# cisco-system-traffic-generator/trex-emu

Measured on AMD Instinct MI355X. Metric: Mpkt/s device-resident rx parse+classify, 1M×64B batch, 1/2/4/8 MI355X, higher is better.
Workload: dtype u8; 1 GPU; B: 1M x 64B untagged IPv4/UDP, 1 ns / 1 client; frames_per_gpu=1048576, frame_bytes_per_gpu=67108864, parallelism=frame shards x1, replicated tables, no collective, tables=replicated, descriptors=keyed (EMURX_DESC_KEYED owner keys, as the device framing walk writes them), table_bytes_per_gpu=109664256, streams=2, batches=8, input_bytes_per_batch=79691840, input_reuse_distance_bytes=637534720

## Files before the change

### include/emu_rx.h

```cpp
#ifndef EMU_RX_H
#define EMU_RX_H

#include <stddef.h>
#include <stdint.h>

#ifdef __cplusplus
extern "C" {
#endif

#define EMURX_ABI_VERSION 6

#define EMURX_OK 0
#define EMURX_EINVAL (-22)
#define EMURX_ENOMEM (-12)
#define EMURX_EEXIST (-17)
#define EMURX_ENOENT (-2)
#define EMURX_EDEVICE (-5)
#define EMURX_ENOSPC (-28)

#define EMURX_ID_NONE 0xFFFFFFFFu

#define EMURX_MAX_FRAME 9216u
#define EMURX_ZMQ_MAGIC 0xBEEFu

// ... 325 lines not shown
    EMURX_LRN_NONE = 0,
    EMURX_LRN_ARP_REQ = 1, EMURX_LRN_ARP_REPLY = 2, EMURX_LRN_ND_NS = 3, EMURX_LRN_ND_NA = 4,
    EMURX_LRN_HOST = 5
};
#define EMURX_LRNK_ARP 1u
#define EMURX_LRNK_ND  2u
#define EMURX_LRNK_ALL 3u
#define EMURX_LRN_INFO_WORDS 8
uint32_t emurx_learn_max_events(const emurx_t* h);
int emurx_learn_dev(emurx_t* h, const uint8_t* d_frames, const emurx_desc* d_desc,
                    const emurx_rec* d_rec, uint32_t n, uint32_t kinds,
                    emurx_learn_ev* d_ev, uint32_t ev_cap,
                    uint8_t* d_outcome, uint64_t* d_info, void* stream);

void emurx_hist_to_counters(const uint64_t hist[2 * EMURX_HIST_BINS], emurx_counters* out);
void emurx_hist_fold(const uint64_t* shards, uint64_t out[2 * EMURX_HIST_BINS]);

int emurx_set_timing(emurx_t* h, uint32_t slots, uint32_t stride);
int emurx_kernel_times(emurx_t* h, float* batch_ms, uint32_t cap, uint32_t* n_out);

const char* emurx_build_id(void);

uint32_t emurx_last_stage(const emurx_t* h);
int32_t emurx_last_txz(const emurx_t* h);

int emurx_copy_ceiling_dev(void* d_dst, const void* d_src, size_t bytes, void* stream);

#define EMURX_MAX_PARTS 8
typedef struct emurx_route_rec {
    emurx_rec rec;
    uint32_t src_index;
    uint32_t src_rank;
} emurx_route_rec;

uint32_t emurx_ns_owner(const uint8_t key[12], uint32_t n_parts);
uint8_t emurx_owner_key(const uint8_t key[12]);
int emurx_desc_keys_dev(emurx_t* h, const uint8_t* d_frames, emurx_desc* d_desc, uint32_t n, void* stream);
int emurx_route_dev(emurx_t* h, const emurx_rec* d_rec, uint32_t n, uint32_t n_parts, uint32_t my_rank,
                    uint32_t cap, emurx_route_rec* d_send, uint32_t* d_send_count, void* stream);
int emurx_classify_route_dev(emurx_t* h, const uint8_t* d_frames, const emurx_desc* d_desc, uint32_t n,
                             const emurx_dev_out* out, uint32_t n_parts, uint32_t my_rank, uint32_t cap,
                             emurx_route_rec* d_send, uint32_t* d_send_count, void* stream);

#define EMURX_TAIL_SHARDS 64u
#define EMURX_TAIL_CURSOR_STRIDE 64u
#define EMURX_LOOKUP_REGION_BYTES(cap, tail_cap) \
// ... 36 lines not shown
```

### trex-emu_amd/csrc/emurx_api.cpp

```cpp
#include <hip/hip_runtime.h>

#include <algorithm>
#include <atomic>
#include <chrono>
#include <array>
#include <cstdio>
#include <cstdlib>
#include <cstring>
#include <new>
#include <string>
#include <vector>

#include "../../include/emu_rx.h"
#include "emurx_kernels.h"
#include "emurx_mirror.h"
#include "emurx_tables.h"

using emurx_host::Blocks;
using emurx_host::Hash;
using emurx_host::Mirror;

namespace {

uint16_t be16(const uint8_t* p) { return (uint16_t)((p[0] << 8) | p[1]); }
// ... 133 lines not shown
    uint32_t txz_calls = 0, txz_last_copy = 0, txz_every = 8, txz_same = 0;
    int last_txz = -1;
    DevBuf<uint8_t> d_rsp;
    DevBuf<uint8_t> d_lrn;
    bool lrn_dirty = false;

    struct RouteScratch {
        hipStream_t st = nullptr;
        bool used = false;
        hipEvent_t done = nullptr;
        DevBuf<uint32_t> cnt, grp, goff;
        DevBuf<uint32_t> tcur;
        void release() {
            cnt.release(); grp.release(); goff.release(); tcur.release();
            if (done) (void)hipEventDestroy(done);
            done = nullptr;
        }
    };
    static constexpr size_t kRouteSets = 4;
    RouteScratch route[kRouteSets];
    uint32_t route_next = 0;

    DevBuf<uint32_t> d_stage_fb;
    PinBuf<uint32_t> stage_fb;
    uint32_t stage_gen = 0, stage_mode = 0;
    bool stage_copy = false, stage_pending = false;
    uint32_t stage_copy_gen = 0;
    uint32_t stage_every = 8, stage_same = 0;
    hipEvent_t stage_ev = nullptr;
    uint32_t stage_bytes = emurx::kStageWide;
    bool stage_tight_ok = false;
    uint32_t last_stage = 0;

    emurx_comm_state* comm = nullptr;

    std::vector<hipEvent_t> ev;
    uint32_t slots = 0, ev_head = 0, ev_count = 0, stride = 1, batch_seq = 0;

    emurx_dev_tables tables() const {
        using namespace emurx_host;
        emurx_dev_tables T{};
        T.ns_tab = d_tab[kTabNs].p;
        T.ns_info = d_nsinfo.p;
        T.mac_tab = d_tab[kTabMac].p;
        T.ip4_tab = d_tab[kTabIp4].p;
        T.ip6_tab = d_tab[kTabIp6].p;
// ... 207 lines not shown
    return EMURX_HIP_OK(hipEventRecord(r->done, st)) ? EMURX_OK : EMURX_EDEVICE;
}

int not_capturing(hipStream_t st) {
    hipStreamCaptureStatus cs = hipStreamCaptureStatusNone;
    if (!EMURX_HIP_OK(hipStreamIsCapturing(st, &cs))) return EMURX_EDEVICE;
    return cs == hipStreamCaptureStatusNone ? EMURX_OK : EMURX_EINVAL;
}

int run_dev(emurx_t* h, const uint8_t* frames, const emurx_desc* desc, uint32_t n, const emurx_dev_out* out,
            hipStream_t st, int kind, const emurx_route_args* rt) {
    int rc;
    if ((rc = not_capturing(st))) return rc;
    if (kind == 1 && (rc = prepare_read(h, st))) return rc;
    emurx_dev_tables T = h->tables();
    const hipEvent_t* ev = nullptr;
    if (h->slots && (h->batch_seq++ % h->stride) == 0) {
        const uint32_t s = h->ev_head;
        ev = &h->ev[2 * s];
        h->ev_head = (s + 1) % h->slots;
        h->ev_count = std::min(h->ev_count + 1, h->slots);
    }
    const uint32_t stage = choose_stage(h);
    int r = emurx_launch_batch(frames, desc, n, T, kind, *out, st, ev, stage, h->d_stage_fb.p, h->stage_gen, rt);
    if (!r) r = stage_copy_back(h, st);
    return r ? EMURX_EDEVICE : EMURX_OK;
}

int check_batch_args(emurx_t* h, const uint8_t* frames, const emurx_desc* desc, uint32_t n,
                     const emurx_dev_out* out) {
    if (!h || !out || !out->hist || (n && (!frames || !desc))) return EMURX_EINVAL;
    if (((uintptr_t)frames & 15) || ((uintptr_t)desc & 7)) return EMURX_EINVAL;
    if (n > h->cfg.max_frames) return EMURX_ENOMEM;
    if (out->qlist && out->qcap < queue_cap(n)) return EMURX_EINVAL;
    return bind(h);
}

int ingest_buffer(emurx_t* h, uint32_t slot, size_t bytes, uint8_t** buf) {
    IngestSlot& s = h->ing[slot];
    if (s.pending || bytes > 0xFFFFFFFFull - 64) return EMURX_EINVAL;
    if (s.h_buf.alloc(bytes + 64) || s.d_buf.alloc(bytes + 64)) return EMURX_ENOMEM;
    *buf = s.h_buf.p;
    return EMURX_OK;
}

bool small_fits(const uint32_t* ctl, uint32_t nmsg, uint32_t n, uint32_t max_tiles, uint32_t trange[EMURX_SMALL_TILES]) {
    if (nmsg > EMURX_SMALL_MSGS || n > std::min<uint32_t>(max_tiles, EMURX_SMALL_TILES) * EMURX_QUEUE_TILE) return false;
// ... 102 lines not shown
        if (emurx_launch_ingest_small(s.h_buf.p, ctl, nmsg, n, h->tables(), s.h_rec.p, s.h_desc.p, s.h_qlist.p,
                                      s.h_stat.p, s.h_qoff.p, s.h_hist.p, s.d_qseg.p, s.d_tcnt.p, s.d_hsmall.p,
                                      s.d_ticket.p, s.h_done.p, (s.seq + 1) & 0x7fffffffu,
                                      h->spin_base_us > 0 ? (uint32_t)((h->spin_base_us + 1e-4 * (double)end) * h->wall_khz / 1000.0) : 0u,
                                      trange, st) ||
            !EMURX_HIP_OK(hipEventRecord(s.done, st)))
            return EMURX_EDEVICE;
        s.seq = (s.seq + 1) & 0x7fffffffu;
        s.small = true;
        s.pending = true;
        s.nmsg = nmsg;
        s.slots = n;
        return EMURX_OK;
    }
    const auto H2D = hipMemcpyHostToDevice, D2H = hipMemcpyDeviceToHost;
    bool ok = EMURX_HIP_OK(hipMemcpyAsync(s.d_ctl.p, ctl, ((size_t)3 * nmsg + 1) * 4, H2D, st));
    if (end) ok = ok && EMURX_HIP_OK(hipMemcpyAsync(s.d_buf.p, s.h_buf.p, end, H2D, st));
    if (!ok) return EMURX_EDEVICE;
    if (emurx_launch_zmq_walk(s.d_buf.p, s.d_ctl.p, nmsg, s.d_desc.p, s.d_stat.p, st)) return EMURX_EDEVICE;
    if (n) {
        const emurx_dev_out o{s.d_rec.p, s.d_qlist.p, (uint32_t)qcap, s.d_tile_cnt.p, s.d_hist.p};
        const uint32_t stage = choose_stage(h);
        if (emurx_launch_batch(s.d_buf.p, s.d_desc.p, n, h->tables(), true, o, st, nullptr, stage,
                               h->d_stage_fb.p, h->stage_gen) ||
            stage_copy_back(h, st))
            return EMURX_EDEVICE;
    }
    if (emurx_launch_queue_pack(s.d_qlist.p, (uint32_t)qcap, s.d_tile_cnt.p, n, s.d_seg_off.p, s.d_packed.p,
                                s.d_qoff.p, s.d_hist.p, s.d_hist_out.p, st))
        return EMURX_EDEVICE;
    ok = EMURX_HIP_OK(hipMemcpyAsync(s.h_res.p, s.d_res.p, s.res_bytes, D2H, st)) &&
         EMURX_HIP_OK(hipEventRecord(s.done, st));
    if (!ok) return EMURX_EDEVICE;
    s.small = false;
    s.pending = true;
    s.nmsg = nmsg;
    s.slots = n;
    return EMURX_OK;
}

bool spin_done(const uint32_t* word, uint32_t seq) {
    const volatile uint32_t* w = word;
    const auto t0 = std::chrono::steady_clock::now();
    for (uint32_t k = 1;; ++k) {
        if ((*w & 0x7fffffffu) == seq) {
            std::atomic_thread_fence(std::memory_order_acquire);
            return true;
// ... 88 lines not shown
}

int emurx_open(const emurx_cfg* cfg, emurx_t** out) {
    if (!cfg || !out || cfg->max_ns == 0 || cfg->max_clients == 0 || cfg->max_frames == 0) return EMURX_EINVAL;
    emurx_t* h = new (std::nothrow) emurx_ctx();
    if (!h) return EMURX_ENOMEM;
    h->cfg = *cfg;
    if (h->cfg.max_bytes == 0) h->cfg.max_bytes = 1u << 20;
    h->host_only = cfg->device < 0;
    try {
        h->m.open(cfg->max_ns, cfg->max_clients);
    } catch (...) {
        delete h;
        return EMURX_ENOMEM;
    }
    if (h->host_only) {
        *out = h;
        return EMURX_OK;
    }
    int rc = bind(h);
    if (rc) { delete h; return rc; }
    if (!EMURX_HIP_OK(hipStreamCreate(&h->stream))) { delete h; return EMURX_EDEVICE; }
    if (const char* e = getenv("EMURX_STAGE")) h->stage_mode = !strcmp(e, "wide") ? 1 : !strcmp(e, "narrow") ? 2 : !strcmp(e, "tight") ? 3 : 0;
    if (const char* e = getenv("EMURX_INGEST_SMALL")) h->ingest_small = strcmp(e, "0") != 0;
    if (const char* e = getenv("EMURX_TXZ"))
        h->txz_mode = !strcmp(e, "wide") ? EMURX_TXZ_WIDE : !strcmp(e, "narrow") ? EMURX_TXZ_NARROW
                    : !strcmp(e, "long") ? EMURX_TXZ_LONG : -1;
    if (const char* e = getenv("EMURX_INGEST_SPIN")) h->ingest_spin = strcmp(e, "0") != 0;
    {
        int khz = 100000;
        if (EMURX_HIP_OK(hipDeviceGetAttribute(&khz, hipDeviceAttributeWallClockRate, cfg->device)) && khz > 0)
            h->wall_khz = (uint32_t)khz;
        if (const char* e = getenv("EMURX_INGEST_SPIN_US")) h->spin_base_us = std::min(std::max(0.0, strtod(e, nullptr)), 1e6);
        const uint32_t cap = emurx_ingest_small_capacity(cfg->device);
        h->small_tiles = std::min<uint32_t>(EMURX_SMALL_TILES, cap);
    }
    if (h->stage_fb.alloc(256) || h->d_stage_fb.alloc(256) ||
        !EMURX_HIP_OK(hipEventCreateWithFlags(&h->stage_ev, hipEventDisableTiming)) ||
        !EMURX_HIP_OK(hipEventCreateWithFlags(&h->ship_ev, hipEventDisableTiming)) ||
        !EMURX_HIP_OK(hipMemset(h->d_stage_fb.p, 0, 256 * sizeof(uint32_t)))) {
        emurx_close(h);
        return EMURX_ENOMEM;
    }
    for (auto& s : h->ring)
        if (!EMURX_HIP_OK(hipEventCreateWithFlags(&s.ev, hipEventDisableTiming))) {
            emurx_close(h);
            return EMURX_EDEVICE;
        }
    memset(h->stage_fb.p, 0, 256 * sizeof(uint32_t));
    if (h->d_lrn.alloc(emurx_lrn_scratch_bytes(cfg->max_frames)) ||
        !EMURX_HIP_OK(hipMemset(h->d_lrn.p, 0, (size_t)emurx_lrn_slots(cfg->max_frames) * 16))) {
        emurx_close(h);
        return EMURX_ENOMEM;
    }
    emurx_t::RouteScratch* rs = nullptr;
    if ((rc = ship_tables(h, h->stream)) || (rc = route_scratch(h, cfg->max_frames, h->stream, &rs)) == EMURX_ENOMEM) {
        emurx_close(h);
        return rc ? rc : EMURX_ENOMEM;
    }
    *out = h;
    return EMURX_OK;
}

// ... 396 lines not shown
    for (int b = 0; b < 2 * EMURX_HIST_BINS; ++b) out[b] = 0;
    if (!shards) return;
    for (int s = 0; s < EMURX_HIST_SHARDS; ++s)
        for (int b = 0; b < 2 * EMURX_HIST_BINS; ++b) out[b] += shards[(size_t)s * 2 * EMURX_HIST_BINS + b];
}

int emurx_set_timing(emurx_t* h, uint32_t slots, uint32_t stride) {
    if (!h) return EMURX_EINVAL;
    int rc = bind(h);
    if (rc) return rc;
    (void)hipDeviceSynchronize();
    for (auto& e : h->ev)
        if (e) (void)hipEventDestroy(e);
    h->ev.assign((size_t)slots * 2, nullptr);
    for (auto& e : h->ev)
        if (!EMURX_HIP_OK(hipEventCreateWithFlags(&e, hipEventDisableSystemFence))) { h->slots = 0; return EMURX_EDEVICE; }
    h->slots = slots;
    h->stride = stride ? stride : 1;
    h->ev_head = h->ev_count = h->batch_seq = 0;
    return EMURX_OK;
}

uint32_t emurx_last_stage(const emurx_t* h) { return h ? h->last_stage : 0; }
int32_t emurx_last_txz(const emurx_t* h) {
    if (!h || h->last_txz < 0) return -1;
    return h->last_txz == EMURX_TXZ_NARROW ? 4608 : h->last_txz == EMURX_TXZ_LONG ? 0 : 6144;
}

int emurx_kernel_times(emurx_t* h, float* batch_ms, uint32_t cap, uint32_t* n_out) {
    if (!h || !n_out || (cap && !batch_ms)) return EMURX_EINVAL;
    *n_out = 0;
    if (!h->slots || !h->ev_count) return EMURX_OK;
    int rc = bind(h);
    if (rc) return rc;
    const uint32_t last = (h->ev_head + h->slots - 1) % h->slots;
    if (!EMURX_HIP_OK(hipEventSynchronize(h->ev[2 * last + 1]))) return EMURX_EDEVICE;
    const uint32_t n = std::min(h->ev_count, cap);
    const uint32_t first = (h->ev_head + h->slots - h->ev_count) % h->slots;
    for (uint32_t k = 0; k < n; ++k) {
        const uint32_t s = (first + (h->ev_count - n) + k) % h->slots;
        if (!EMURX_HIP_OK(hipEventElapsedTime(&batch_ms[k], h->ev[2 * s], h->ev[2 * s + 1])))
            return EMURX_EDEVICE;
    }
    *n_out = n;
    h->ev_count = 0;
    return EMURX_OK;
// ... 164 lines not shown
```

### trex-emu_amd/csrc/emurx_kernels.h

```cpp
#pragma once
#include <hip/hip_runtime.h>

#include <cstdio>
#include <cstdlib>
#include <tuple>
#include <type_traits>
#include <utility>

#include "../../include/emu_rx.h"
#include "emurx_tables.h"

inline bool emurx_hip_ok(hipError_t e, const char* file, int line) {
    if (e == hipSuccess) return true;
    static const bool dbg = getenv("EMURX_DEBUG") != nullptr;
    if (dbg) fprintf(stderr, "emurx: HIP error at %s:%d: %s\n", file, line, hipGetErrorString(e));
    return false;
}
#define EMURX_HIP_OK(x) emurx_hip_ok((x), __FILE__, __LINE__)

template <typename... P, typename... A>
inline hipError_t emurx_launch(void (*k)(P...), dim3 grid, dim3 block, size_t lds, hipStream_t st, A&&... a) {
    static_assert(sizeof...(P) == sizeof...(A), "kernel argument count");
    std::tuple<std::decay_t<P>...> args{std::forward<A>(a)...};
    return std::apply(
        [&](auto&... e) {
            void* p[] = {(void*)&e...};
            return hipLaunchKernel((const void*)k, grid, block, p, lds, st);
        },
        args);
}

namespace emurx {
constexpr uint32_t kStageWide = 7168, kStageNarrow = 6144, kStageTight = 5120;
}

struct emurx_route_args {
    uint32_t parts, rank, cap;
    uint32_t* cnt;
    uint32_t* grp;
    const uint32_t* goff;
    emurx_lookup_rec* send;
    uint32_t tcap;
    uint32_t* tcur;
    uint32_t* count;
    uint32_t tup_on;
};
int emurx_launch_batch(const uint8_t* frames, const emurx_desc* desc, uint32_t n,
                       const emurx_dev_tables& T, int kind, const emurx_dev_out& out,
                       hipStream_t st, const hipEvent_t* ev, uint32_t stage, uint32_t* fb, uint32_t gen,
                       const emurx_route_args* rt = nullptr);

struct emurx_delta {
    uint64_t dst;
    uint64_t pad;
    uint32_t w[16];
};
int emurx_launch_apply(const emurx_delta* d, uint32_t n, hipStream_t st);

int emurx_launch_route(const emurx_rec* rec, uint32_t n, uint32_t n_parts, uint32_t my_rank, uint32_t cap,
                       emurx_route_rec* send, uint32_t* send_count, uint32_t* tile_cnt, uint32_t* grp,
                       uint32_t* grp_off, hipStream_t st, bool counted = false);
int emurx_launch_owner_count(const uint8_t* frames, const emurx_desc* desc, uint32_t n, uint32_t n_parts,
                             uint32_t* send_count, uint32_t* tile_cnt, uint32_t* grp, uint32_t* grp_off,
                             uint32_t* tcur, hipStream_t st);
int emurx_launch_desc_keys(const uint8_t* frames, emurx_desc* desc, uint32_t n, hipStream_t st);
int emurx_launch_lookup(const emurx_lookup_rec* recv, const uint32_t* recv_count, uint32_t n_parts, uint32_t cap,
                        uint32_t tcap, const emurx_dev_tables& T, emurx_route_rec* out, uint32_t* flow,
                        hipStream_t st);

int emurx_launch_zmq_walk(const uint8_t* buf, const uint32_t* ctl, uint32_t nmsg, emurx_desc* desc,
                          uint32_t* msg_stat, hipStream_t st, bool keys = true);
#ifndef EMURX_SMALL_TILES
#define EMURX_SMALL_TILES 256
// ... 42 lines not shown
```

### trex-emu_amd/csrc/emurx_kernels.hip

```cpp
#include <hip/hip_runtime.h>

#include "../../include/emu_rx.h"
#include "emurx_kernels.h"
#include "emurx_parse.h"
#include "emurx_tables.h"

namespace emurx {

static_assert(EMURX_QUEUE_TILE == kBlock, "one frame per lane per tile");


template <bool kNt>
__device__ __forceinline__ void glds16(const uint4* src, uint4* dst_wave_base) {
    __builtin_amdgcn_global_load_lds(src, (__attribute__((address_space(3))) void*)dst_wave_base, 16, 0,
                                     kNt ? 2 : 0);
}
__device__ __forceinline__ void wait_vm0() { __builtin_amdgcn_s_waitcnt(0x0F70); }

#ifndef EMURX_STAMP
#define EMURX_STAMP 0
#endif
#if EMURX_STAMP
__device__ unsigned long long* g_stamp;
#define STAMP(k) \
    do { if constexpr (EMURX_STAMP) st_[k] = __builtin_amdgcn_s_memtime(); } while (0)
#else
#define STAMP(k) do {} while (0)
#endif

#ifndef EMURX_TOL_PREFETCH
#define EMURX_TOL_PREFETCH 1
#endif
struct RxArgs {
    const uint8_t* frames;
    const emurx_desc* desc;
    uint32_t n;
    emurx_dev_tables T;
    emurx_rec* rec;
    uint32_t* qlist;
    uint32_t qcap;
    uint32_t* tile_cnt;
    unsigned long long* hist;
    uint32_t* flow;
    uint32_t* fb;
    uint32_t gen;
    emurx_route_args rt;
};

__device__ __forceinline__ uint2 load_desc(const emurx_desc* __restrict__ desc, uint32_t n, uint32_t i) {
    return i < n ? *reinterpret_cast<const uint2*>(desc + i) : make_uint2(0, EMURX_DESC_HOLE << 24);
}

#ifndef EMURX_WIN_NT
#define EMURX_WIN_NT 0
#endif
struct Stage {
    uint32_t start, nvec;
    bool staged;
};
template <uint32_t kStage>
__device__ __forceinline__ Stage stage_issue(const uint8_t* __restrict__ frames, uint2 dd, uint32_t lane, uint4* wslab) {
    constexpr uint32_t kWinVec = kStage / 16 / kWave;
    const bool valid = (dd.y >> 24) != EMURX_DESC_HOLE;
    const uint32_t off = dd.x, len = dd.y & 0xffff;
    const uint32_t lo = wave_min_u32(valid ? off : 0xffffffffu);
    const uint32_t hi = wave_max_u32(valid ? off + len : 0u);
    Stage sg;
    sg.start = lo & ~15u;
// ... 72 lines not shown
#endif
    const uint32_t i = tile * EMURX_QUEUE_TILE + tid;
    if (lane < 16) L.wcnt[wv][lane] = 0;
    if (lane < EMURX_MAX_PARTS) L.rcnt[wv][lane] = 0;
    if (kKind == 2 && wv == 0) {
        const TileOffLoads t = EMURX_TOL_PREFETCH ? tol : tile_offsets_issue(rt.cnt, rt.goff, rt.parts, tile, lane);
        tile_offsets_sum(t, rt.parts, lane, L.toff, [](uint32_t v) { return wave_sum_u32(v); });
    }
    const bool valid = (dd.y >> 24) != EMURX_DESC_HOLE;
    const uint32_t off = dd.x, len = dd.y & 0xffff, vport = (dd.y >> 16) & 0xff;
    if (a.fb && (tile & 63) == 0 && lane == 0) {
        const uint32_t bytes = sg.nvec * 16;
        const uint32_t mid = bytes > kStageNarrow && bytes <= kStageWide;
        a.fb[((tile >> 6) & 63) * kWaves + wv] = (a.gen << 3) | ((bytes > kStageTight) << 2) | ((sg.nvec > 0) << 1) | mid;
    }

    Rec r;
    r.dlen = 0;
    uint4* const wslab = reinterpret_cast<uint4*>(const_cast<uint32_t*>(slab)) + wv * (kStage / 16);
    uint4* lhead = wslab + lane * 2;
    uint4* ltail = wslab + kWave * 2 + lane * 3;
    static_assert(kStage >= kWave * (32 + 48), "a wave's lookup heads and tails fit its slab");
    uint32_t tun = 0;
    auto classify_parked = [&](const auto& s) {
        if constexpr (kParkRec) {
            typedef std::decay_t<decltype(s)> S;
            volatile uint32_t* pa = &L.csum[wv][lane];
            volatile uint32_t* pb = &L.park[wv][lane];
            *pa = r.l4 | (r.l7 << 16);
            static_assert(EMURX_FLAG_RTALERT < 8 && EMURX_ST_PANIC_MBUF < 32, "flags and status share the parked byte");
            *pb = r.l7len | (r.nh << 16) | (r.flags << 24) | (r.status << 27);
            r.flags = 0;
            if (r.status == EMURX_ST_OK) {
                const LKey k = make_key(s, len, r);
                const uint32_t l3 = r.l3;
                auto again = [&]() {
                    if constexpr (std::is_same<S, WinSrc>::value) {
                        uint32_t o2 = off, l2 = lane;
                        asm volatile("" : "+v"(o2), "+v"(l2));
                        const uint32_t h2 = (uint32_t)((uintptr_t)(a.frames + o2) & 15);
                        return WinSrc{reinterpret_cast<const uint8_t*>(slab), slab, wv * kStage + l2 * 16, h2,
                                      (uint32_t)min(kWinVec * 16 - h2, len), a.frames + o2};
                    } else {
                        return s;
                    }
                };
                resolve(T, r, k,
                        [&](uint32_t cid) {
                            Rec q;
                            q.l3 = l3;
                            q.l4 = *pa & 0xffffu;
                            q.nh = (*pb >> 16) & 0xffu;
                            return flow_probe(T, get_tuple(again(), len, q), cid);
                        },
                        [&]() {
                            const S s2 = again();
                            return make_uint3(le32(s2, 0), s2.u8(4) | (s2.u8(5) << 8), s2.u8(l3 + 8) == 0xff);
                        });
            }
            const uint32_t wa = *pa, wb = *pb;
            r.l4 = wa & 0xffffu;
            r.l7 = wa >> 16;
            r.l7len = wb & 0xffffu;
            r.nh = (wb >> 16) & 0xffu;
            r.flags |= (wb >> 24) & 7u;
            r.status = wb >> 27;
        }
    };
    if (sg.staged) {
        if (valid) {
            LdsSrc s{reinterpret_cast<const uint8_t*>(slab), slab, wv * kStage + (off - sg.start)};
            parse_flat(s, len, vport, T.cb_mask, r);
            STAMP(3);
            if constexpr (kParkRec) classify_parked(s);
            else if (kClassify) classify(s, len, T, r);
            if (kKind == 2) tun = pack_lookup(s, len, r, i, r.status == EMURX_ST_OK, rt.tup_on, lhead, ltail);
        }
    } else {
        const uint32_t head = (uint32_t)((uintptr_t)(a.frames + off) & 15);
        WinSrc s{reinterpret_cast<const uint8_t*>(slab), slab, wv * kStage + lane * 16, head,
                 min(kWinVec * 16 - head, len), a.frames + off};
        if (valid) parse_packet(s, len, vport, T.cb_mask, r);
        coop_checksum_rows(r, a.frames + off, L.csum[wv]);
        STAMP(3);
        if constexpr (kParkRec) {
            if (valid) classify_parked(s);
        } else if (valid && kClassify) {
            classify(s, len, T, r);
        }
        if (kKind == 2 && valid) tun = pack_lookup(s, len, r, i, r.status == EMURX_ST_OK, rt.tup_on, lhead, ltail);
    }
    STAMP(4);
    uint32_t rd = 0xffu, rrank = 0, tofs = 0, tlead = 0, tb = 0;
    const uint32_t shard = tile & (EMURX_TAIL_SHARDS - 1);
    if constexpr (kKind == 2) {
        const uint32_t pad = dd.y >> 24;
        rd = !valid ? 0xffu
             : (pad & EMURX_DESC_KEYED) ? emurx_owner_of_key(pad, rt.parts)
                                        : emurx_owner(emurx_tk_hash(r.vport, r.vlan0, r.vlan1), rt.parts);
        uint64_t rl = __ballot(rd != 0xffu);
        while (rl) {
            const uint32_t lead = (uint32_t)__ffsll((long long)rl) - 1;
            const uint32_t d2 = (uint32_t)__builtin_amdgcn_readlane((int)rd, (int)lead);
            const uint64_t m = __ballot(rd == d2);
            const uint64_t m1 = __ballot(rd == d2 && tun == 1), m3 = __ballot(rd == d2 && tun == 3);
            if (rd == d2) {
                rrank = mbcnt(m);
                tofs = mbcnt(m1) + 3 * mbcnt(m3);
            }
            if (lane == lead) L.rcnt[wv][d2] = (uint32_t)__popcll(m);
            if (m1 | m3) {
                const uint32_t tl = (uint32_t)__ffsll((long long)(m1 | m3)) - 1;
                if (lane == tl)
                    tb = atomicAdd(&rt.tcur[(d2 * EMURX_TAIL_SHARDS + shard) * EMURX_TAIL_CURSOR_STRIDE],
                                   (uint32_t)(__popcll(m1) + 3 * __popcll(m3)));
// ... 196 lines not shown
#else
    tile_body<kKind, kStage>(a, tile, dd, sg, slab, L, tol);
#endif
}

__global__ __launch_bounds__(kBlock) void k_apply(const emurx_delta* __restrict__ d, uint32_t n) {
    const uint32_t i = blockIdx.x * kBlock + threadIdx.x, e = i >> 2, q = i & 3;
    if (e >= n) return;
    const uint4 v = reinterpret_cast<const uint4*>(d[e].w)[q];
    reinterpret_cast<uint4*>((uintptr_t)d[e].dst)[q] = v;
}

}

int emurx_launch_apply(const emurx_delta* d, uint32_t n, hipStream_t st) {
    using namespace emurx;
    if (!n) return 0;
    return EMURX_HIP_OK(emurx_launch(k_apply, dim3((n * 4 + kBlock - 1) / kBlock), dim3(kBlock), 0, st, d, n)) ? 0 : -1;
}

int emurx_launch_batch(const uint8_t* frames, const emurx_desc* desc, uint32_t n,
                       const emurx_dev_tables& T, int kind, const emurx_dev_out& out,
                       hipStream_t st, const hipEvent_t* ev, uint32_t stage, uint32_t* fb, uint32_t gen,
                       const emurx_route_args* rt) {
    using namespace emurx;
    hipError_t e = hipSuccess;
#ifndef EMURX_RX_LDS_PAD
#define EMURX_RX_LDS_PAD 0
#endif
    if (ev && !EMURX_HIP_OK(hipEventRecord(ev[0], st))) return -1;
    if (n) {
        const uint32_t ntiles = (n + EMURX_QUEUE_TILE - 1) / EMURX_QUEUE_TILE;
        unsigned long long* hist = reinterpret_cast<unsigned long long*>(out.hist);
        const emurx_route_args none{};
        const RxArgs args{frames, desc, n, T, out.rec, out.qlist, out.qcap, out.tile_cnt, hist, out.flow, fb, gen,
                          rt ? *rt : none};
        const bool narrow = stage == kStageNarrow, tight = stage == kStageTight;
        auto k = kind == 1 ? (tight ? k_rx<1, kStageTight> : narrow ? k_rx<1, kStageNarrow> : k_rx<1, kStageWide>)
               : kind == 2 ? (tight ? k_rx<2, kStageTight> : narrow ? k_rx<2, kStageNarrow> : k_rx<2, kStageWide>)
                           : (tight ? k_rx<0, kStageTight> : narrow ? k_rx<0, kStageNarrow> : k_rx<0, kStageWide>);
        e = emurx_launch(k, dim3(ntiles), dim3(kBlock), EMURX_RX_LDS_PAD, st, args);
    }
    if (!EMURX_HIP_OK(e)) return -1;
    return ev && !EMURX_HIP_OK(hipEventRecord(ev[1], st)) ? -1 : 0;
}

namespace emurx {
constexpr int kCopyInFlight = 4;
constexpr int kCopyGrid = 16384;
__global__ __launch_bounds__(kBlock) void k_copy(uint4* __restrict__ dst, const uint4* __restrict__ src, size_t nv) {
    typedef unsigned v4 __attribute__((ext_vector_type(4)));
    const size_t stride = (size_t)gridDim.x * kBlock * kCopyInFlight;
    for (size_t base = (size_t)blockIdx.x * kBlock * kCopyInFlight + threadIdx.x; base < nv; base += stride) {
        v4 x[kCopyInFlight];
#pragma unroll
        for (int k = 0; k < kCopyInFlight; ++k) {
            const size_t i = base + (size_t)k * kBlock;
            x[k] = i < nv ? __builtin_nontemporal_load(reinterpret_cast<const v4*>(src) + i) : v4{0, 0, 0, 0};
        }
// ... 24 lines not shown
```

### trex-emu_amd/csrc/emurx_parse.h

```cpp
#pragma once
#include <hip/hip_runtime.h>

#include "../../include/emu_rx.h"
#include "emurx_kernels.h"
#include "emurx_tables.h"

namespace emurx {

constexpr int kWave = 64;
constexpr int kBlock = 256;
constexpr int kWaves = kBlock / kWave;

typedef unsigned emurx_v4u __attribute__((ext_vector_type(4)));
__device__ __forceinline__ uint4 gld16(const void* p) {
    const emurx_v4u v = *(const __attribute__((address_space(1))) emurx_v4u*)p;
    return make_uint4(v.x, v.y, v.z, v.w);
}
typedef unsigned emurx_v3u __attribute__((ext_vector_type(3)));
__device__ __forceinline__ uint3 gld12(const void* p) {
    const emurx_v3u v = *(const __attribute__((address_space(1))) emurx_v3u*)p;
    return make_uint3(v.x, v.y, v.z);
}
__device__ __forceinline__ uint32_t gld4(const void* p) { return *(const __attribute__((address_space(1))) uint32_t*)p; }
__device__ __forceinline__ uint32_t gld1(const void* p) { return *(const __attribute__((address_space(1))) uint8_t*)p; }
// ... 1290 lines not shown
    Bucket ce{};
    if (p.ctab) ce = ld_bucket(p.ctab, p.cbk);
#if EMURX_FLATRES == 2
    if (__ballot(k.key != (uint32_t)__builtin_amdgcn_readfirstlane((int)k.key)) == 0)
        resolve_done(T, r, k, p, ce, flow, dmac);
    else
        resolve_done_flat(T, r, k, p, ce, flow, dmac);
#elif EMURX_FLATRES
    resolve_done_flat(T, r, k, p, ce, flow, dmac);
#else
    resolve_done(T, r, k, p, ce, flow, dmac);
#endif
}
template <class Flow>
__device__ __forceinline__ void resolve(const emurx_dev_tables& T, Rec& r, const LKey& k, Flow flow) {
    resolve(T, r, k, flow, [&]() { return make_uint3(k.dlo, k.dhi, k.mc6); });
}

template <class S>
__device__ __forceinline__ void classify(const S& s, uint32_t len, const emurx_dev_tables& T, Rec& r) {
    if (r.status != EMURX_ST_OK) return;
    const LKey k = make_key(s, len, r);
    resolve(T, r, k, [&](uint32_t cid) { return flow_probe(T, get_tuple(s, len, r), cid); });
}

__device__ __forceinline__ bool lk_transport(uint32_t cb) { return cb == EMURX_CB_TCP || cb == EMURX_CB_UDP; }
__device__ __forceinline__ bool lk_ip6key(uint32_t key) { return key == kIp6 || key == kEui; }
__device__ __forceinline__ uint32_t vlan_code(uint32_t v) {
    return v == 0 ? 0u : ((((v >> 16) == 0x8100u) ? 1u : 2u) << 12) | (v & 0xfffu);
}
__device__ __forceinline__ uint32_t vlan_word(uint32_t c) {
    const uint32_t t = (c >> 12) & 3u;
    return t == 0 ? 0u : ((t == 1 ? 0x8100u : 0x88A8u) << 16) | (c & 0xfffu);
}
__device__ __forceinline__ uint2 eui_mac(uint32_t w2, uint32_t w3) {
    return make_uint2(((w2 & 0xff) ^ 2) | (((w2 >> 8) & 0xff) << 8) | (((w2 >> 16) & 0xff) << 16) | (((w3 >> 8) & 0xff) << 24),
                      ((w3 >> 16) & 0xff) | ((w3 >> 24) << 8));
}
__device__ __forceinline__ uint32_t lk_tail_units(uint32_t w4) {
    const uint32_t key = (w4 >> 28) & 7u;
    if (((w4 >> 20) & 31u) != EMURX_ST_OK) return 0;
    if (lk_ip6key(key)) return 1;
    return (w4 >> 31) ? (((w4 >> 26) & 1u) ? 3u : 1u) : 0u;
}
template <class S>
__device__ __forceinline__ uint32_t pack_lookup(const S& s, uint32_t len, const Rec& r, uint32_t frame, bool ok,
// ... 99 lines not shown
```

### trex-emu_amd/emurx/abi.py

```python
from __future__ import annotations

import ctypes as C
import os
from pathlib import Path

import numpy as np

PKG_ROOT = Path(__file__).resolve().parent.parent
REPO_ROOT = PKG_ROOT.parent
LIB_PATH = PKG_ROOT / "lib" / "libemurx.so"

EMURX_OK = 0
EMURX_EINVAL, EMURX_ENOMEM, EMURX_EEXIST, EMURX_ENOENT = -22, -12, -17, -2
EMURX_EDEVICE, EMURX_ENOSPC = -5, -28
EMURX_ECOMM = -71
COMM_ID_BYTES = 128
XCH_EQUAL, XCH_PAYLOAD, XCH_ROUTE = 0, 1, 2
ID_NONE = 0xFFFFFFFF
MAX_FRAME = 9216

CB_NAMES = ["arp", "icmp", "igmp", "dhcp", "dhcpsrv", "dhcpv6", "mdns", "tcp", "udp",
            "icmpv6", "eapol", "ppp"]
(CB_ARP, CB_ICMP, CB_IGMP, CB_DHCP, CB_DHCPSRV, CB_DHCPV6, CB_MDNS, CB_TCP, CB_UDP,
 CB_ICMPV6, CB_EAPOL, CB_PPP) = range(12)
# ... 143 lines not shown
    ("emurx_ns_add", C.c_int, [_P, _U8P, C.c_uint32, C.c_uint32]),
    ("emurx_ns_remove", C.c_int, [_P, _U8P]),
    ("emurx_ns_set_plugins", C.c_int, [_P, C.c_uint32, C.c_uint32]),
    ("emurx_client_add", C.c_int, [_P, C.c_uint32, C.c_uint32, _U8P, _U8P, _U8P, _U8P, C.c_uint32]),
    ("emurx_clients_add", C.c_int, [_P, _P, C.c_uint32, C.POINTER(C.c_uint32)]),
    ("emurx_client_remove", C.c_int, [_P, C.c_uint32, _U8P]),
    ("emurx_client_set_plugins", C.c_int, [_P, C.c_uint32, C.c_uint32]),
    ("emurx_client_update_ipv4", C.c_int, [_P, C.c_uint32, _U8P]),
    ("emurx_client_update_ipv6", C.c_int, [_P, C.c_uint32, _U8P]),
    ("emurx_client_update_dipv6", C.c_int, [_P, C.c_uint32, _U8P]),
    ("emurx_client_set_ra", C.c_int, [_P, C.c_uint32, _U8P, C.c_uint8]),
    ("emurx_sync", C.c_int, [_P, _P]),
    ("emurx_rx_stream", C.c_int, [_P, _U8P, C.c_size_t, _P, _P, C.c_uint32,
                                  C.POINTER(C.c_uint32), _P, C.POINTER(Counters)]),
    ("emurx_classify_dev", C.c_int, [_P, _P, _P, C.c_uint32, C.POINTER(DevOut), _P]),
    ("emurx_parse_dev", C.c_int, [_P, _P, _P, C.c_uint32, C.POINTER(DevOut), _P]),
    ("emurx_zmq_descriptors", C.c_int, [_U8P, C.c_size_t, _P, C.c_uint32,
                                        C.POINTER(C.c_uint32), C.POINTER(C.c_int)]),
    ("emurx_hist_to_counters", None, [_P, C.POINTER(Counters)]),
    ("emurx_hist_fold", None, [_P, _P]),
    ("emurx_set_timing", C.c_int, [_P, C.c_uint32, C.c_uint32]),
    ("emurx_kernel_times", C.c_int, [_P, _P, C.c_uint32, C.POINTER(C.c_uint32)]),
    ("emurx_last_stage", C.c_uint32, [_P]),
    ("emurx_last_txz", C.c_int32, [_P]),
    ("emurx_copy_ceiling_dev", C.c_int, [_P, _P, C.c_size_t, _P]),
    ("emurx_ns_owner", C.c_uint32, [_U8P, C.c_uint32]),
    ("emurx_owner_key", C.c_uint8, [_U8P]),
    ("emurx_desc_keys_dev", C.c_int, [_P, _P, _P, C.c_uint32, _P]),
    ("emurx_route_dev", C.c_int, [_P, _P, C.c_uint32, C.c_uint32, C.c_uint32, C.c_uint32, _P, _P, _P]),
    ("emurx_classify_route_dev", C.c_int, [_P, _P, _P, C.c_uint32, C.POINTER(DevOut), C.c_uint32, C.c_uint32,
                                           C.c_uint32, _P, _P, _P]),
    ("emurx_parse_route_dev", C.c_int, [_P, _P, _P, C.c_uint32, C.POINTER(DevOut), C.c_uint32, C.c_uint32,
                                        C.c_uint32, C.c_uint32, _P, _P, _P]),
    ("emurx_lookup_dev", C.c_int, [_P, _P, _P, C.c_uint32, C.c_uint32, C.c_uint32, _P, _P, _P]),
    ("emurx_zmq_walk_dev", C.c_int, [_P, _P, _P, C.c_uint32, _P, _P, C.c_uint32, _P]),
    ("emurx_set_partition", C.c_int, [_P, C.c_uint32, C.c_uint32]),
    ("emurx_table_gen", C.c_uint64, [_P]),
    ("emurx_recs_stale", C.c_int, [_P, _P, C.c_uint32, C.c_uint64, _P]),
    ("emurx_image_lookup", C.c_int, [_P, C.c_uint32, _P, C.POINTER(C.c_uint32)]),
    ("emurx_image_probe", C.c_int, [_P, C.c_uint32, _P, _P]),
    ("emurx_image_check", C.c_int, [_P, C.POINTER(C.c_uint64)]),
    ("emurx_table_stats", C.c_int, [_P, C.POINTER(C.c_uint64), C.POINTER(C.c_uint64), C.POINTER(C.c_uint64)]),
    ("emurx_ingest_buffer", C.c_int, [_P, C.c_uint32, C.c_size_t, C.POINTER(C.c_void_p)]),
    ("emurx_ingest_submit", C.c_int, [_P, C.c_uint32, _P, C.c_uint32]),
    ("emurx_ingest_wait", C.c_int, [_P, C.c_uint32, C.POINTER(IngestResult)]),
    ("emurx_ingest_stream", C.c_int, [_P, C.c_uint32, C.POINTER(C.c_void_p)]),
    ("emurx_tx_checksum_dev", C.c_int, [_P, _P, _P, C.c_uint32, _P, _P]),
    ("emurx_tx_zmq_dev", C.c_int, [_P, _P, _P, C.c_uint32, _P, C.c_uint64, _P, _P, _P]),
    ("emurx_respond_dev", C.c_int, [_P, _P, _P, _P, C.c_uint32, _P, C.c_uint64, _P, _P, _P, _P, _P]),
    ("emurx_respond_kinds_dev", C.c_int, [_P, _P, _P, _P, C.c_uint32, C.c_uint32, _P, C.c_uint64, _P, _P, _P, _P, _P]),
    ("emurx_learn_max_events", C.c_uint32, [_P]),
    ("emurx_learn_dev", C.c_int, [_P, _P, _P, _P, C.c_uint32, C.c_uint32, _P, C.c_uint32, _P, _P, _P]),
    ("emurx_flow_add", C.c_int, [_P, C.c_uint32, _U8P, C.c_uint32, C.c_uint32]),
    ("emurx_flow_remove", C.c_int, [_P, C.c_uint32, _U8P, C.c_uint32]),
    ("emurx_server_add", C.c_int, [_P, C.c_uint32, C.c_uint16, C.c_uint8]),
    ("emurx_server_remove", C.c_int, [_P, C.c_uint32, C.c_uint16, C.c_uint8]),
    ("emurx_client_set_transport", C.c_int, [_P, C.c_uint32, C.c_int]),
    ("emurx_comm_unique_id", C.c_int, [_P]),
    ("emurx_comm_init", C.c_int, [_P, _P, C.c_uint32, C.c_uint32]),
    ("emurx_comm_init_all", C.c_int, [_P, C.c_uint32]),
    ("emurx_comm_destroy", C.c_int, [_P]),
    ("emurx_comm_info", C.c_int, [_P, C.POINTER(C.c_uint32), C.POINTER(C.c_uint32)]),
    ("emurx_comm_library", C.c_int, [C.c_char_p, C.c_size_t]),
    ("emurx_group_start", C.c_int, []),
    ("emurx_group_end", C.c_int, []),
    ("emurx_exchange_dev", C.c_int, [_P, _P, _P, _P, _P, C.c_uint32, C.c_uint32, C.c_uint32,
                                     C.POINTER(C.c_uint64), _P]),
]

_lib = None


def load(path: str | os.PathLike | None = None):
    global _lib
    if _lib is not None and path is None:
        return _lib
    p = Path(path) if path else Path(os.environ.get("EMURX_LIB", LIB_PATH))
    if not p.exists():
        raise OSError(f"libemurx.so not built at {p}: run `make -C {PKG_ROOT}` "
                      "(there is no CPU fallback for the product path)")
    lib = C.CDLL(str(p), mode=C.RTLD_GLOBAL)
    for name, res, args in SIGNATURES:
        fn = getattr(lib, name)
        fn.restype = res
        fn.argtypes = args
    if path is None:
        _lib = lib
        built, tree = lib.emurx_build_id().decode(), source_id()
        import sys
        print(f"emurx: {p} built from source tree {built}" +
              ("" if tree in (built, None) else f" -- STALE: this tree is {tree}"), file=sys.stderr)
    return lib


def source_id() -> str | None:
    import hashlib
    src = ["emurx_kernels.hip", "emurx_route.hip", "emurx_ingest.hip", "emurx_tx.hip", "emurx_txzmq.hip",
           "emurx_respond.hip", "emurx_learn.hip", "emurx_api.cpp", "emurx_mirror.cpp", "emurx_comm.cpp"]
    hdr = ["emurx_kernels.h", "emurx_tables.h", "emurx_parse.h", "emurx_mirror.h", "emurx_rsp_dev.h"]
    files = [PKG_ROOT / "csrc" / f for f in src + hdr] + [REPO_ROOT / "include" / "emu_rx.h", PKG_ROOT / "Makefile"]
    h = hashlib.sha1()
    try:
        for f in files:
            h.update(f.read_bytes())
    except OSError:
        return None
# ... 19 lines not shown
```

### trex-emu_amd/emurx/rx.py

```python
from __future__ import annotations

import ctypes as C

import numpy as np

from . import abi


def _u8(x, n):
    if x is None:
        return None
    a = np.frombuffer(bytes(x), dtype=np.uint8).copy()
    if a.size != n:
        raise ValueError(f"expected {n} bytes, got {a.size}")
    return a


def _p(a):
    return None if a is None else a.ctypes.data


class RxPath:

    def __init__(self, device: int = 0, max_ns: int = 4096, max_clients: int = 65536,
# ... 127 lines not shown
        out = abi.DevOut(_addr(rec), _addr(qlist), qcap, _addr(tile_cnt), _addr(hist), _addr(flow))
        fn = self.lib.emurx_classify_dev if classify else self.lib.emurx_parse_dev
        args = (self.h, _addr(frames), _addr(desc), n, C.byref(out), _stream(stream))

        def call():
            rc = fn(*args)
            if rc:
                abi.check(rc, "classify_dev")
        call.keep = out
        return call

    def set_timing(self, slots: int = 1024, stride: int = 1):
        return abi.check(self.lib.emurx_set_timing(self.h, slots, stride), "set_timing")

    def kernel_times(self, cap: int = 1 << 16):
        a = np.zeros(cap, np.float32)
        n = C.c_uint32()
        abi.check(self.lib.emurx_kernel_times(self.h, _p(a), cap, C.byref(n)), "kernel_times")
        return a[: n.value]

    def last_stage(self) -> int:
        return int(self.lib.emurx_last_stage(self.h))

    def last_txz(self) -> int:
        return int(self.lib.emurx_last_txz(self.h))

    def ingest_buffer(self, slot: int, nbytes: int) -> np.ndarray:
        p = C.c_void_p()
        abi.check(self.lib.emurx_ingest_buffer(self.h, slot, nbytes, C.byref(p)), "ingest_buffer")
        return np.ctypeslib.as_array(C.cast(p, C.POINTER(C.c_uint8)), shape=(max(nbytes, 1),))[:nbytes]

    def ingest_submit(self, slot: int, msgs) -> None:
        a = np.asarray(msgs)
        a = np.ascontiguousarray(a).view(np.uint32) if a.dtype.names else np.asarray(msgs, dtype=np.uint32)
        m = np.ascontiguousarray(a).reshape(-1, 2)
        abi.check(self.lib.emurx_ingest_submit(self.h, slot, _p(m) if len(m) else None, len(m)),
                  "ingest_submit")

    def ingest_stream(self, slot: int) -> int:
        p = C.c_void_p()
        abi.check(self.lib.emurx_ingest_stream(self.h, slot, C.byref(p)), "ingest_stream")
        return int(p.value)

    def ingest_wait(self, slot: int, copy: bool = True) -> dict:
        r = abi.IngestResult()
        abi.check(self.lib.emurx_ingest_wait(self.h, slot, C.byref(r)), "ingest_wait")
# ... 249 lines not shown
```

Measured before the change: 52560 Mpkt/s.

## Add wave-uniform fast path for parse and classify of same-shape IPv4 frames

Adds a wave-level check that all frames in a wave share the same ethertype, tag count and L4 protocol with a simple IPv4 header. When they do, a specialized parser runs with wave-uniform offsets and a word-aligned checksum loop, and a simplified namespace/client hash lookup skips the general classify path. The goal is to cut divergent, generic parse and lookup work on homogeneous traffic. It adds ballot checks and some duplicated logic, enabled by default and switchable with EMURX_UNIFORM, plus a sampled feedback word per wave for diagnostics.

```diff
diff --git a/include/emu_rx.h b/include/emu_rx.h
--- a/include/emu_rx.h
+++ b/include/emu_rx.h
@@ -371,6 +371,11 @@
 const char* emurx_build_id(void);
 
 uint32_t emurx_last_stage(const emurx_t* h);
+#define EMURX_UNI_WORDS 256
+#define EMURX_UNI_PARSE 1u
+#define EMURX_UNI_LOOKUP 2u
+#define EMURX_UNI_SAMPLED 4u
+int emurx_last_uniform(emurx_t* h, uint32_t words[EMURX_UNI_WORDS]);
 int32_t emurx_last_txz(const emurx_t* h);
 
 int emurx_copy_ceiling_dev(void* d_dst, const void* d_src, size_t bytes, void* stream);
diff --git a/trex-emu_amd/csrc/emurx_api.cpp b/trex-emu_amd/csrc/emurx_api.cpp
--- a/trex-emu_amd/csrc/emurx_api.cpp
+++ b/trex-emu_amd/csrc/emurx_api.cpp
@@ -179,6 +179,7 @@
     uint32_t route_next = 0;
 
     DevBuf<uint32_t> d_stage_fb;
+    bool uniform = true;
     PinBuf<uint32_t> stage_fb;
     uint32_t stage_gen = 0, stage_mode = 0;
     bool stage_copy = false, stage_pending = false;
@@ -432,7 +433,7 @@
         h->ev_count = std::min(h->ev_count + 1, h->slots);
     }
     const uint32_t stage = choose_stage(h);
-    int r = emurx_launch_batch(frames, desc, n, T, kind, *out, st, ev, stage, h->d_stage_fb.p, h->stage_gen, rt);
+    int r = emurx_launch_batch(frames, desc, n, T, kind, *out, st, ev, stage, h->d_stage_fb.p, h->stage_gen, h->uniform, rt);
     if (!r) r = stage_copy_back(h, st);
     return r ? EMURX_EDEVICE : EMURX_OK;
 }
@@ -581,7 +582,7 @@
         const emurx_dev_out o{s.d_rec.p, s.d_qlist.p, (uint32_t)qcap, s.d_tile_cnt.p, s.d_hist.p};
         const uint32_t stage = choose_stage(h);
         if (emurx_launch_batch(s.d_buf.p, s.d_desc.p, n, h->tables(), true, o, st, nullptr, stage,
-                               h->d_stage_fb.p, h->stage_gen) ||
+                               h->d_stage_fb.p, h->stage_gen, h->uniform) ||
             stage_copy_back(h, st))
             return EMURX_EDEVICE;
     }
@@ -716,6 +717,7 @@
     if (rc) { delete h; return rc; }
     if (!EMURX_HIP_OK(hipStreamCreate(&h->stream))) { delete h; return EMURX_EDEVICE; }
     if (const char* e = getenv("EMURX_STAGE")) h->stage_mode = !strcmp(e, "wide") ? 1 : !strcmp(e, "narrow") ? 2 : !strcmp(e, "tight") ? 3 : 0;
+    if (const char* e = getenv("EMURX_UNIFORM")) h->uniform = strcmp(e, "0") != 0;
     if (const char* e = getenv("EMURX_INGEST_SMALL")) h->ingest_small = strcmp(e, "0") != 0;
     if (const char* e = getenv("EMURX_TXZ"))
         h->txz_mode = !strcmp(e, "wide") ? EMURX_TXZ_WIDE : !strcmp(e, "narrow") ? EMURX_TXZ_NARROW
@@ -729,10 +731,10 @@
         const uint32_t cap = emurx_ingest_small_capacity(cfg->device);
         h->small_tiles = std::min<uint32_t>(EMURX_SMALL_TILES, cap);
     }
-    if (h->stage_fb.alloc(256) || h->d_stage_fb.alloc(256) ||
+    if (h->stage_fb.alloc(256) || h->d_stage_fb.alloc(2 * emurx::kFbWords) ||
         !EMURX_HIP_OK(hipEventCreateWithFlags(&h->stage_ev, hipEventDisableTiming)) ||
         !EMURX_HIP_OK(hipEventCreateWithFlags(&h->ship_ev, hipEventDisableTiming)) ||
-        !EMURX_HIP_OK(hipMemset(h->d_stage_fb.p, 0, 256 * sizeof(uint32_t)))) {
+        !EMURX_HIP_OK(hipMemset(h->d_stage_fb.p, 0, 2 * emurx::kFbWords * sizeof(uint32_t)))) {
         emurx_close(h);
         return EMURX_ENOMEM;
     }
@@ -1175,6 +1177,17 @@
 }
 
 uint32_t emurx_last_stage(const emurx_t* h) { return h ? h->last_stage : 0; }
+int emurx_last_uniform(emurx_t* h, uint32_t words[EMURX_UNI_WORDS]) {
+    static_assert(EMURX_UNI_WORDS == emurx::kFbWords, "one path word per sampled wave");
+    if (!h || !words) return EMURX_EINVAL;
+    if (bind(h)) return EMURX_EDEVICE;
+    if (!EMURX_HIP_OK(hipDeviceSynchronize()) ||
+        !EMURX_HIP_OK(hipMemcpy(words, h->d_stage_fb.p + emurx::kFbWords, EMURX_UNI_WORDS * sizeof(uint32_t), hipMemcpyDeviceToHost)))
+        return EMURX_EDEVICE;
+    for (uint32_t i = 0; i < EMURX_UNI_WORDS; ++i)
+        words[i] = h->stage_gen && (words[i] >> 2) == h->stage_gen ? EMURX_UNI_SAMPLED | (words[i] & 3u) : 0u;
+    return EMURX_OK;
+}
 int32_t emurx_last_txz(const emurx_t* h) {
     if (!h || h->last_txz < 0) return -1;
     return h->last_txz == EMURX_TXZ_NARROW ? 4608 : h->last_txz == EMURX_TXZ_LONG ? 0 : 6144;
diff --git a/trex-emu_amd/csrc/emurx_kernels.h b/trex-emu_amd/csrc/emurx_kernels.h
--- a/trex-emu_amd/csrc/emurx_kernels.h
+++ b/trex-emu_amd/csrc/emurx_kernels.h
@@ -32,6 +32,7 @@
 
 namespace emurx {
 constexpr uint32_t kStageWide = 7168, kStageNarrow = 6144, kStageTight = 5120;
+constexpr uint32_t kFbWords = 256;
 }
 
 struct emurx_route_args {
@@ -48,7 +49,7 @@
 int emurx_launch_batch(const uint8_t* frames, const emurx_desc* desc, uint32_t n,
                        const emurx_dev_tables& T, int kind, const emurx_dev_out& out,
                        hipStream_t st, const hipEvent_t* ev, uint32_t stage, uint32_t* fb, uint32_t gen,
-                       const emurx_route_args* rt = nullptr);
+                       bool uniform, const emurx_route_args* rt = nullptr);
 
 struct emurx_delta {
     uint64_t dst;
diff --git a/trex-emu_amd/csrc/emurx_kernels.hip b/trex-emu_amd/csrc/emurx_kernels.hip
--- a/trex-emu_amd/csrc/emurx_kernels.hip
+++ b/trex-emu_amd/csrc/emurx_kernels.hip
@@ -44,6 +44,7 @@
     uint32_t* flow;
     uint32_t* fb;
     uint32_t gen;
+    uint32_t uniform;
     emurx_route_args rt;
 };
 
@@ -162,7 +163,8 @@
     uint4* ltail = wslab + kWave * 2 + lane * 3;
     static_assert(kStage >= kWave * (32 + 48), "a wave's lookup heads and tails fit its slab");
     uint32_t tun = 0;
-    auto classify_parked = [&](const auto& s) {
+    auto classify_parked = [&](const auto& s, bool try_uni) {
+        bool done = false;
         if constexpr (kParkRec) {
             typedef std::decay_t<decltype(s)> S;
             volatile uint32_t* pa = &L.csum[wv][lane];
@@ -171,7 +173,10 @@
             static_assert(EMURX_FLAG_RTALERT < 8 && EMURX_ST_PANIC_MBUF < 32, "flags and status share the parked byte");
             *pb = r.l7len | (r.nh << 16) | (r.flags << 24) | (r.status << 27);
             r.flags = 0;
-            if (r.status == EMURX_ST_OK) {
+            if constexpr (std::is_same<S, LdsSrc>::value) {
+                if (try_uni) done = classify_uniform(s, T, r);
+            }
+            if (!done && r.status == EMURX_ST_OK) {
                 const LKey k = make_key(s, len, r);
                 const uint32_t l3 = r.l3;
                 auto again = [&]() {
@@ -206,14 +211,26 @@
             r.flags |= (wb >> 24) & 7u;
             r.status = wb >> 27;
         }
+        return done;
     };
+    uint32_t uni = 0;
     if (sg.staged) {
+        LdsSrc s{reinterpret_cast<const uint8_t*>(slab), slab, wv * kStage + (valid ? off - sg.start : 0u)};
+        bool try_uni = false;
+        if (a.uniform) {
+            const UniShape u = uniform_shape(s, valid, len);
+            if (u.ok) {
+                parse_uniform(s, vport, T.cb_mask, u, r);
+                uni = 1;
+                if constexpr (kParkRec) try_uni = true;
+                else if constexpr (kClassify) uni |= classify_uniform(s, T, r) ? 2u : 0u;
+            }
+        }
         if (valid) {
-            LdsSrc s{reinterpret_cast<const uint8_t*>(slab), slab, wv * kStage + (off - sg.start)};
-            parse_flat(s, len, vport, T.cb_mask, r);
+            if (!(uni & 1)) parse_flat(s, len, vport, T.cb_mask, r);
             STAMP(3);
-            if constexpr (kParkRec) classify_parked(s);
-            else if (kClassify) classify(s, len, T, r);
+            if constexpr (kParkRec) uni |= classify_parked(s, try_uni) ? 2u : 0u;
+            else if (kClassify && !(uni & 2)) classify(s, len, T, r);
             if (kKind == 2) tun = pack_lookup(s, len, r, i, r.status == EMURX_ST_OK, rt.tup_on, lhead, ltail);
         }
     } else {
@@ -224,13 +241,14 @@
         coop_checksum_rows(r, a.frames + off, L.csum[wv]);
         STAMP(3);
         if constexpr (kParkRec) {
-            if (valid) classify_parked(s);
+            if (valid) classify_parked(s, false);
         } else if (valid && kClassify) {
             classify(s, len, T, r);
         }
         if (kKind == 2 && valid) tun = pack_lookup(s, len, r, i, r.status == EMURX_ST_OK, rt.tup_on, lhead, ltail);
     }
     STAMP(4);
+    if (a.fb && (tile & 63) == 0 && lane == 0) a.fb[kFbWords + ((tile >> 6) & 63) * kWaves + wv] = (a.gen << 2) | uni;
     uint32_t rd = 0xffu, rrank = 0, tofs = 0, tlead = 0, tb = 0;
     const uint32_t shard = tile & (EMURX_TAIL_SHARDS - 1);
     if constexpr (kKind == 2) {
@@ -473,7 +491,7 @@
 int emurx_launch_batch(const uint8_t* frames, const emurx_desc* desc, uint32_t n,
                        const emurx_dev_tables& T, int kind, const emurx_dev_out& out,
                        hipStream_t st, const hipEvent_t* ev, uint32_t stage, uint32_t* fb, uint32_t gen,
-                       const emurx_route_args* rt) {
+                       bool uniform, const emurx_route_args* rt) {
     using namespace emurx;
     hipError_t e = hipSuccess;
 #ifndef EMURX_RX_LDS_PAD
@@ -485,7 +503,7 @@
         unsigned long long* hist = reinterpret_cast<unsigned long long*>(out.hist);
         const emurx_route_args none{};
         const RxArgs args{frames, desc, n, T, out.rec, out.qlist, out.qcap, out.tile_cnt, hist, out.flow, fb, gen,
-                          rt ? *rt : none};
+                          uniform ? 1u : 0u, rt ? *rt : none};
         const bool narrow = stage == kStageNarrow, tight = stage == kStageTight;
         auto k = kind == 1 ? (tight ? k_rx<1, kStageTight> : narrow ? k_rx<1, kStageNarrow> : k_rx<1, kStageWide>)
                : kind == 2 ? (tight ? k_rx<2, kStageTight> : narrow ? k_rx<2, kStageNarrow> : k_rx<2, kStageWide>)
diff --git a/trex-emu_amd/csrc/emurx_parse.h b/trex-emu_amd/csrc/emurx_parse.h
--- a/trex-emu_amd/csrc/emurx_parse.h
+++ b/trex-emu_amd/csrc/emurx_parse.h
@@ -1336,6 +1336,107 @@
     if (r.status != EMURX_ST_OK) return;
     const LKey k = make_key(s, len, r);
     resolve(T, r, k, [&](uint32_t cid) { return flow_probe(T, get_tuple(s, len, r), cid); });
+}
+
+__device__ __forceinline__ uint32_t wave_first(uint32_t v) { return (uint32_t)__builtin_amdgcn_readfirstlane((int)v); }
+struct UniShape {
+    uint32_t tags, l3, nh;
+    uint32_t totlen;
+    bool ok;
+};
+__device__ __forceinline__ UniShape uniform_shape(const LdsSrc& s, bool valid, uint32_t len) {
+    auto is_tag = [](uint32_t x) { return x == 0x8100 || x == 0x88A8; };
+    UniShape u{0, 0, 0, 0, false};
+    const uint32_t e0 = be16(s, 12), e0w = wave_first(e0);
+    if (__ballot(!valid || e0 != e0w)) return u;
+    uint32_t nt = 0;
+    if (is_tag(e0w)) nt = is_tag(be16(s, 16)) ? 2u : 1u;
+    u.tags = wave_first(nt);
+    u.l3 = 14 + 4 * u.tags;
+    const uint32_t et = be16(s, u.l3 - 2), b0 = s.u8(u.l3), frag = be16(s, u.l3 + 6), nh = s.u8(u.l3 + 9);
+    u.totlen = be16(s, u.l3 + 2);
+    u.nh = wave_first(nh);
+    const uint32_t need = u.nh == 6 ? 40u : 28u;
+    const bool pass = valid && nt == u.tags && et == 0x0800 && b0 == 0x45 && (frag & 0x3fff) == 0 && nh == u.nh &&
+                      len == u.l3 + u.totlen && u.totlen >= need;
+    u.ok = (u.nh == 6 || u.nh == 17) && __ballot(pass) == ~0ull;
+    return u;
+}
+__device__ __forceinline__ uint32_t span_sum_wave(const LdsSrc& s, uint32_t at, uint32_t n) {
+    const uint32_t a = s.base + at;
+    const uint32_t sa = wave_first(a & 3), sn = wave_first(n);
+    if (__ballot((a & 3) != sa || n != sn)) return s.sum(at, n);
+    const uint32_t e = sa + sn, last = (e - 1) >> 2;
+    const uint32_t hm = 0xffffffffu << (8 * sa), tm = 0xffffffffu >> (8 * ((0u - e) & 3));
+    const uint32_t* w = s.b32 + (a >> 2);
+    uint32_t acc = sad16(w[0] & hm, 0), j = 1;
+    for (; j + 4 <= last; j += 4) {
+        const uint32_t x0 = w[j], x1 = w[j + 1], x2 = w[j + 2], x3 = w[j + 3];
+        acc = sad16(x3, sad16(x2, sad16(x1, sad16(x0, acc))));
+    }
+    for (; j < last; ++j) acc = sad16(w[j], acc);
+    return sad16(w[last] & tm, acc);
+}
+__device__ __forceinline__ void parse_uniform(const LdsSrc& s, uint32_t vport, uint32_t cb_mask, const UniShape& u, Rec& r) {
+    const uint32_t L3 = u.l3, L4 = L3 + 20, l4len = u.totlen - 20;
+    r.ns = EMURX_ID_NONE; r.cl = EMURX_ID_NONE;
+    r.vlan0 = u.tags >= 1 ? (be32(s, 12) & 0xffff0fffu) : 0u;
+    r.vlan1 = u.tags == 2 ? (be32(s, 16) & 0xffff0fffu) : 0u;
+    r.vport = vport;
+    r.l3 = L3;
+    r.flags = 0;
+    r.dlen = 0;
+    r.flow = EMURX_FLOW_NONE;
+    const bool hok = csum_ok(s.template sum_fixed<20>(L3), s.at(L3), 0);
+    const uint32_t pcs = be_domain(s.template sum_fixed<8>(L3 + 12), s.at(L3 + 12)) + u.nh + l4len;
+    const bool cs = csum_ok(span_sum_wave(s, L4, l4len), s.at(L4), pcs);
+    uint32_t st, cb, l7, l7len;
+    if (u.nh == 17) {
+        const bool ucs = (s.u8(L4 + 6) | s.u8(L4 + 7)) != 0;
+        st = ucs && !cs ? EMURX_ST_UDP_CS : EMURX_ST_OK;
+        l7len = (l4len - 8) & 0xffff;
+        l7 = st == EMURX_ST_OK ? L4 + 8 : 0u;
+        const uint32_t src = be16(s, L4), dst = be16(s, L4 + 2);
+        cb = dst == 5353 ? EMURX_CB_MDNS
+           : (src == 67 && dst == 68) ? EMURX_CB_DHCP
+           : (dst == 67 && (src == 67 || src == 68)) ? EMURX_CB_DHCPSRV : EMURX_CB_UDP;
+    } else {
+        const uint32_t tcplen = (s.u8(L4 + 12) >> 4) << 2;
+        const bool fits = l4len >= tcplen;
+        st = !fits ? EMURX_ST_TCP_TOO_SHORT : !cs ? EMURX_ST_TCP_CS : EMURX_ST_OK;
+        l7len = fits ? ((l4len - tcplen) & 0xffff) : 0u;
+        l7 = fits ? ((L4 + tcplen) & 0xffff) : 0u;
+        cb = EMURX_CB_TCP;
+    }
+    st = hok ? st : (uint32_t)EMURX_ST_IPV4_CS;
+    r.l4 = hok ? L4 : 0u;
+    r.nh = hok ? u.nh : 0u;
+    r.l7 = hok ? l7 : 0u;
+    r.l7len = hok ? l7len : 0u;
+    r.proto = st == EMURX_ST_OK ? cb : (uint32_t)EMURX_CB_NONE;
+    r.status = st != EMURX_ST_OK ? st : ((cb_mask >> cb) & 1u) ? (uint32_t)EMURX_ST_OK : (uint32_t)EMURX_ST_NOT_SUPPORTED;
+}
+__device__ __forceinline__ bool classify_uniform(const LdsSrc& s, const emurx_dev_tables& T, Rec& r) {
+    const bool plain = r.status == EMURX_ST_OK && (r.proto == EMURX_CB_UDP || r.proto == EMURX_CB_TCP);
+    if (__ballot(!plain)) return false;
+    const uint32_t lo = le32(s, 0), hi = s.u8(4) | (s.u8(5) << 8);
+    const uint32_t tk = emurx_tk_hash(r.vport, r.vlan0, r.vlan1);
+    const uint4 x = gld16(T.ns_tab + (size_t)(tk & T.ns_mask) * EMURX_BUCKET_WORDS);
+    const uint4 y = gld16(T.mac_tab + (size_t)(emurx_mac_hash(tk, lo, hi) & T.mac_mask) * EMURX_BUCKET_WORDS);
+    const uint32_t plug = 1u << EMURX_PLUG_TRANSPORT;
+    static_assert(kCbPluginTab[EMURX_CB_UDP] == EMURX_PLUG_TRANSPORT && kCbPluginTab[EMURX_CB_TCP] == EMURX_PLUG_TRANSPORT,
+                  "udp and tcp check the transport plugin");
+    const bool ns_hit = x.w != EMURX_EMPTY && (x.x & 0xffffu) == r.vport && x.y == r.vlan0 && x.z == r.vlan1 &&
+                        ((x.x >> 16) & plug);
+    const bool cl_hit = y.w != EMURX_EMPTY && y.x == x.w && y.y == lo && (y.z & 0xffffu) == hi;
+    const bool flows = T.ft_on && ((y.z >> 16) & EMURX_CPL_CTX);
+    if (__ballot(!((lo | hi) != 0 && ns_hit && cl_hit && !flows))) return false;
+    r.ns = x.w;
+    r.cl = y.w;
+    const bool has = (y.z >> 16) & plug;
+    set_lk(r, has ? EMURX_LK_CLIENT : EMURX_LK_CLIENT_NO_PLUGIN);
+    r.flow = has ? EMURX_FLOW_NO_CTX : r.flow;
+    return true;
 }
 
 __device__ __forceinline__ bool lk_transport(uint32_t cb) { return cb == EMURX_CB_TCP || cb == EMURX_CB_UDP; }
diff --git a/trex-emu_amd/emurx/abi.py b/trex-emu_amd/emurx/abi.py
--- a/trex-emu_amd/emurx/abi.py
+++ b/trex-emu_amd/emurx/abi.py
@@ -189,6 +189,7 @@
     ("emurx_set_timing", C.c_int, [_P, C.c_uint32, C.c_uint32]),
     ("emurx_kernel_times", C.c_int, [_P, _P, C.c_uint32, C.POINTER(C.c_uint32)]),
     ("emurx_last_stage", C.c_uint32, [_P]),
+    ("emurx_last_uniform", C.c_int, [_P, _P]),
     ("emurx_last_txz", C.c_int32, [_P]),
     ("emurx_copy_ceiling_dev", C.c_int, [_P, _P, C.c_size_t, _P]),
     ("emurx_ns_owner", C.c_uint32, [_U8P, C.c_uint32]),
@@ -235,6 +236,9 @@
                                      C.POINTER(C.c_uint64), _P]),
 ]
 
+OPTIONAL = {"emurx_last_uniform"}
+UNI_WORDS, UNI_PARSE, UNI_LOOKUP, UNI_SAMPLED = 256, 1, 2, 4
+
 _lib = None
 
 
@@ -248,7 +252,10 @@
                       "(there is no CPU fallback for the product path)")
     lib = C.CDLL(str(p), mode=C.RTLD_GLOBAL)
     for name, res, args in SIGNATURES:
-        fn = getattr(lib, name)
+        fn = getattr(lib, name, None)
+        if fn is None and name in OPTIONAL and "EMURX_LIB" in os.environ and path is None:
+            continue
+        fn = fn or getattr(lib, name)
         fn.restype = res
         fn.argtypes = args
     if path is None:
diff --git a/trex-emu_amd/emurx/rx.py b/trex-emu_amd/emurx/rx.py
--- a/trex-emu_amd/emurx/rx.py
+++ b/trex-emu_amd/emurx/rx.py
@@ -173,6 +173,11 @@
     def last_stage(self) -> int:
         return int(self.lib.emurx_last_stage(self.h))
 
+    def last_uniform(self) -> np.ndarray:
+        w = np.zeros(abi.UNI_WORDS, np.uint32)
+        abi.check(self.lib.emurx_last_uniform(self.h, _p(w)), "last_uniform")
+        return w
+
     def last_txz(self) -> int:
         return int(self.lib.emurx_last_txz(self.h))
 
```

Result: faster. 57920 Mpkt/s (median of 6 runs) (+10.2%).
